# liubingqi7/audio-motion-avatar

Hardware: AMD Instinct MI355X
Metric: rendered frames/sec @512x512, 10k Gaussians (static triplane decode + SMPL-X LBS + tile rasterize) (higher is better)
Workload: dtype f32 (LBS blend-shape product: fp16 x 2 split operands with fp32 accumulation, fp32-equivalent; everything else plain fp32)

## Files before the change

audio-motion-avatar_amd/csrc/rasterizer.hip:

```cpp
#include <algorithm>
#include <cmath>
#include <cstddef>
#include <cstdlib>

#include "amav_common.h"
#include "decode_quad.h"
#include "raster_project.h"
#include "raster_workspace.h"

namespace amav {
namespace raster {

#ifndef AMAV_BIN_ABLATE
#define AMAV_BIN_ABLATE 0
#endif
#ifndef AMAV_ABLATE
#define AMAV_ABLATE 0
#endif
constexpr int kRenderWavesPerSimd = 4;
constexpr int kFusedMinFrames = 96;
constexpr int kSortCap = 512;
constexpr int kBigLdsCap = 2048;
constexpr int kBigBlocks = 1280;

constexpr int kQueues = 8;
constexpr int kBuckets = 17;

__host__ __device__ inline int bucket_of(int n) { return n > 512 ? 0 : 16 - (n - 1) / 32; }

struct Status {
    long long total;
    long long max_frame;
    long long emitted;
    int overflow;
    int big_count;
    int qcount[kQueues][kBuckets];
    int nempty;
    int next[kQueues][32];
};

struct Buffers {
    float4 *geom;
    uint4 *rectd;
    int *tile_off;
    unsigned long long *keys;
    unsigned *sorted;
    int *big_list;
    int4 *queue;
    int *empty_list;
    int *slice_counts;
    Status *status;
};

static inline int bin_slices(int F) { return F >= kFusedMinFrames ? 0 : std::min(16, std::max(1, (256 + F - 1) / F)); }

static inline size_t queue_capacity(int F, int gx, int gy) { return (size_t)F * ((gy + kQueues - 1) / kQueues) * gx; }

static Buffers carve(void *ws, int F, int N, int gx, int gy, long long cap, size_t *bytes) {
    const int T = gx * gy;
    Carver c(ws);
    Buffers b;
    b.status = c.take<Status>(1);
    b.geom = c.take<float4>(((size_t)F * N + 1024) * 3);
    b.rectd = c.take<uint4>((size_t)F * N + 1024);
    b.tile_off = c.take<int>((size_t)F * (T + 1));
    b.keys = c.take<unsigned long long>((size_t)cap);
    b.sorted = c.take<unsigned>((size_t)cap);
    b.big_list = c.take<int>((size_t)F * T);
    b.queue = c.take<int4>((size_t)kQueues * kBuckets * queue_capacity(F, gx, gy));
    b.empty_list = c.take<int>((size_t)F * T);
    b.slice_counts = c.take<int>((size_t)F * bin_slices(F) * T);
    if (bytes) *bytes = c.total();
    return b;
}

struct Params {
    int F, N, H, W, gx, gy, T;
    amav_attr means3d, rotations, scales, opacities, colors;
    const float *view, *proj, *tanfov;
    float bg[3];
    float scale_modifier;
    int apply_activations;
    float scale_bias, scale_max, opacity_bias;
    int antialiasing, clamp_output;
    float *out_rgba;
    float *out_inv_depth;
    int *out_radii;
    long long cap_per_frame;
    int qcap;
    unsigned long long *stamps;
    int *wire_header, *wire_frame_counts, *wire_offsets;
    unsigned char *wire_payload;
    int wire_cap;
    unsigned wire_bg;
    int stash;
    int slices;
    Buffers buf;
    struct {
        const float4 *proj;
        const float *vertices;
        const int *idx4;
        const float *transl;
        const float4 *wpoint;
        float4 *out;
        float radius;
        int R, V;
        int rec_lds;
    } dec;
};

__device__ __forceinline__ int opaque(int x) {
    asm volatile("" : "+v"(x));
    return x;
}
__device__ __forceinline__ int lane_now() {
    int l;
    asm volatile("v_mbcnt_lo_u32_b32 %0, -1, 0\n\tv_mbcnt_hi_u32_b32 %0, -1, %0" : "=v"(l));
    return l;
}
__device__ __forceinline__ unsigned zero_now() {
    unsigned z;
    asm volatile("v_mov_b32 %0, 0" : "=v"(z));
    return z;
}

__device__ __forceinline__ void wave_sync() {
    __builtin_amdgcn_fence(__ATOMIC_RELEASE, "wavefront");
    __builtin_amdgcn_wave_barrier();
    __builtin_amdgcn_fence(__ATOMIC_ACQUIRE, "wavefront");
}

struct GaussRec {
    float4 r0, r1, r2, r3;
};

template <bool kPacked>
__device__ __forceinline__ GaussRec load_gaussian(const Params &p, int f, int i) {
    GaussRec g;
    if (kPacked) {
        const float4 *rec = reinterpret_cast<const float4 *>(at(p.means3d, f, i));
        g.r0 = rec[0], g.r1 = rec[1], g.r2 = rec[2], g.r3 = rec[3];
    } else {
        const float *m_ = at(p.means3d, f, i), *q_ = at(p.rotations, f, i), *s_ = at(p.scales, f, i);
        const float *c_ = at(p.colors, f, i);
        g.r0 = make_float4(m_[0], m_[1], m_[2], at(p.opacities, f, i)[0]);
        g.r1 = make_float4(q_[0], q_[1], q_[2], q_[3]);
        g.r2 = make_float4(s_[0], s_[1], s_[2], 0.f);
        g.r3 = make_float4(c_[0], c_[1], c_[2], 0.f);
    }
    return g;
}

struct FrameCamera {
    float vm[16], pm[16];
    float tanx, tany;
};
__device__ __forceinline__ FrameCamera load_camera(const Params &p, int f) {
    FrameCamera c;
    auto uniform = [](float v) { return __uint_as_float(__builtin_amdgcn_readfirstlane(__float_as_uint(v))); };
#pragma unroll
    for (int k = 0; k < 16; ++k) c.vm[k] = uniform(p.view[f * 16 + k]), c.pm[k] = uniform(p.proj[f * 16 + k]);
    c.tanx = uniform(p.tanfov[2 * f]), c.tany = uniform(p.tanfov[2 * f + 1]);
    return c;
}

__device__ __forceinline__ uint4 preprocess_one(const Params &p, const GaussRec &rec, const FrameCamera &cam,
                                                int &upstream_tiles, float4 (&g)[3]) {
#pragma clang fp contract(off)
    const float *vm = cam.vm, *pm = cam.pm;
    const float tanx = cam.tanx, tany = cam.tany;
    uint4 rd = make_uint4(0u, 0u, 0u, 0u);
    const float4 rec0 = rec.r0, rec1 = rec.r1, rec2 = rec.r2, rec3 = rec.r3;
    const float px3 = rec0.x, py3 = rec0.y, pz3 = rec0.z;
    const ViewPoint v = view_point(vm, px3, py3, pz3);
    const float vx = v.x, vy = v.y, vz = v.z;
    if (!(vz > 0.2f)) return rd;
    const ClipPoint cp = clip_point(pm, px3, py3, pz3);
    const float ppx = cp.ppx, ppy = cp.ppy;

    const float r = rec1.x, x = rec1.y, y = rec1.z, z = rec1.w;
    float s0 = rec2.x, s1 = rec2.y, s2 = rec2.z;
    float opacity = rec0.w;
    float c0 = rec3.x, c1 = rec3.y, c2 = rec3.z;
    if (p.apply_activations) {
        float e;
        s0 = scale_act(s0, p.scale_bias, p.scale_max, e);
        s1 = scale_act(s1, p.scale_bias, p.scale_max, e);
        s2 = scale_act(s2, p.scale_bias, p.scale_max, e);
        opacity = opacity_act(opacity, p.opacity_bias);
        c0 = fminf(fmaxf(c0, 0.0f), 1.0f);
        c1 = fminf(fmaxf(c1, 0.0f), 1.0f);
        c2 = fminf(fmaxf(c2, 0.0f), 1.0f);
    }
    s0 *= p.scale_modifier;
    s1 *= p.scale_modifier;
    s2 *= p.scale_modifier;

    const Cov3 cv = cov3d(r, x, y, z, s0, s1, s2);

    const float focal_x = (float)p.W / (2.0f * tanx), focal_y = (float)p.H / (2.0f * tany);
    const float limx = 1.3f * tanx, limy = 1.3f * tany;
    const float tz = vz;
    const float tx = fminf(limx, fmaxf(-limx, vx / tz)) * tz;
    const float ty = fminf(limy, fmaxf(-limy, vy / tz)) * tz;
    const float J00 = focal_x / tz, J02 = -(focal_x * tx) / (tz * tz);
    const float J11 = focal_y / tz, J12 = -(focal_y * ty) / (tz * tz);
    float T0[3], T1[3];
#pragma unroll
    for (int b = 0; b < 3; ++b) {
        T0[b] = J00 * vm[b * 4 + 0] + J02 * vm[b * 4 + 2];
        T1[b] = J11 * vm[b * 4 + 1] + J12 * vm[b * 4 + 2];
    }
    const Cov2 cov = cov2d(cv.S, T0, T1);
    float ca = cov.ca;
    const float cb = cov.cb;
    float cc = cov.cc;

    const float det_cov = ca * cc - cb * cb;
    ca += 0.3f;
    cc += 0.3f;
    const float det = ca * cc - cb * cb;
    float h_scale = 1.0f;
    if (p.antialiasing) h_scale = sqrtf(fmaxf(0.000025f, det_cov / det));
    if (!(det > 0.0f)) return rd;
    const float det_inv = 1.0f / det;
    const float mid = 0.5f * (ca + cc);
    const float root = sqrtf(fmaxf(0.1f, mid * mid - det));
    const float my_radius = ceilf(3.0f * sqrtf(fmaxf(mid + root, mid - root)));
    const float pix_x = ((ppx + 1.0f) * (float)p.W - 1.0f) * 0.5f;
    const float pix_y = ((ppy + 1.0f) * (float)p.H - 1.0f) * 0.5f;
    const int rx0 = min(p.gx, max(0, (int)((pix_x - my_radius) / (float)kTile)));
    const int ry0 = min(p.gy, max(0, (int)((pix_y - my_radius) / (float)kTile)));
    const int rx1 = min(p.gx, max(0, (int)((pix_x + my_radius + (float)(kTile - 1)) / (float)kTile)));
    const int ry1 = min(p.gy, max(0, (int)((pix_y + my_radius + (float)(kTile - 1)) / (float)kTile)));
    if ((rx1 - rx0) * (ry1 - ry0) <= 0) return rd;

    const float op = opacity * h_scale;
    const float tau = 2.0f * logf(255.0f * op);
    float bx = -1e30f, by = -1e30f;
    if (tau > 0.0f) {
        bx = sqrtf(tau * ca) * 1.001f + 0.01f;
        by = sqrtf(tau * cc) * 1.001f + 0.01f;
    }
    upstream_tiles = (rx1 - rx0) * (ry1 - ry0);
    int cx0 = 1, cx1 = 0, cy0 = 1, cy1 = 0;
    if (tau > 0.0f) {
        cx0 = max(rx0, (int)floorf((pix_x - bx) / (float)kTile));
// ... 702 lines not shown
                   (base + c[4]) | ((base + c[5]) << 16), (base + c[6]) | ((base + c[7]) << 16));
    if (lane == 0) cnt[kBuckets512 / 2] = (unsigned)n;
    wave_sync();
    unsigned st[KPL], sz[KPL];
#pragma unroll
    for (int m = 0; m < KPL; ++m) {
        st[m] = (cnt[b[m] >> 1] >> (16 * (b[m] & 1))) & 0xffffu;
        const int nb = b[m] + 1;
        sz[m] = ((cnt[nb >> 1] >> (16 * (nb & 1))) & 0xffffu) - st[m];
        if (lane + 64 * m < n) slice[st[m] + pos[m]] = k[m];
    }
    wave_sync();
#pragma unroll
    for (int m = 0; m < KPL; ++m) {
        unsigned r = pos[m];
        if (lane + 64 * m < n && sz[m] > 1u) {
            r = 0;
            for (unsigned j = 0; j < sz[m]; ++j) r += (unsigned)(slice[st[m] + j] < k[m]);
        }
        pos[m] = st[m] + r;
    }
    wave_sync();
#pragma unroll
    for (int m = 0; m < KPL; ++m)
        if (lane + 64 * m < n) order[pos[m]] = (unsigned)k[m];
    wave_sync();
    return true;
}

__device__ __attribute__((noinline)) void wave_bitonic_sort(unsigned long long *a, unsigned *order, int n, int lane) {
    const int lp = 32 - __builtin_clz(n - 1);
    const int half = 1 << (lp - 1);
    auto cmpswap = [&](int lo, int hi) {
        if (hi < n) {
            const unsigned long long x = a[lo], y = a[hi];
            if (x > y) {
                a[lo] = y;
                a[hi] = x;
            }
        }
    };
    for (int lk = 1; lk <= lp; ++lk) {
        const int k = 1 << lk, hk = k >> 1;
        for (int c = lane; c < half; c += 64) {
            const int base = (c >> (lk - 1)) << lk, o = c & (hk - 1);
            cmpswap(base + o, base + k - 1 - o);
        }
        wave_sync();
        for (int lj = lk - 2; lj >= 0; --lj) {
            const int j = 1 << lj;
            for (int c = lane; c < half; c += 64) {
                const int lo = ((c >> lj) << (lj + 1)) + (c & (j - 1));
                cmpswap(lo, lo + j);
            }
            wave_sync();
        }
    }
    unsigned id[kSortCap / 64];
#pragma unroll
    for (int m = 0; m < kSortCap / 64; ++m) id[m] = (lane + 64 * m < n) ? (unsigned)a[lane + 64 * m] : 0u;
    wave_sync();
#pragma unroll
    for (int m = 0; m < kSortCap / 64; ++m)
        if (lane + 64 * m < n) order[lane + 64 * m] = id[m];
    wave_sync();
}

#define AMAV_BLEND_GEO(k0, k1, qa, qb, qc, L)           \
    "v_fma_f32 v92, -" qb ", %[ly], " k0 "\n\t"                                                                    \
    "v_fma_f32 v93, -" qc ", %[ly], " k1 "\n\t"                                                                    \
    "v_fma_f32 v92, -" qa ", %[lx], v92\n\t"                                                                       \
    "v_fma_f32 v92, -v92, v92, " L "\n\t"
#define AMAV_BLEND_REST(r, g, b, d, col_wait, DEPTH)                                                               \
    "v_fma_f32 v92, -v93, v93, v92\n\t"                                                                            \
    "v_exp_f32_e32 v92, v92\n\t"                                                                                   \
    "s_nop 0\n\t"                                                                                                  \
    "v_min_f32_e32 v92, 0x3f7d70a4, v92\n\t"                                                    \
    "v_cmp_le_f32_e32 vcc, 0x3b808081, v92\n\t"                                               \
    "s_nop 1\n\t"                                                                                                  \
    "v_cndmask_b32_e32 v92, 0, v92, vcc\n\t"                                       \
    "v_fma_f32 v93, -v92, %[T], %[T]\n\t"                                                   \
    "v_cmp_gt_f32_e32 vcc, 0x38d1b717, v93\n\t"                                          \
    "v_mul_f32_e32 v94, v92, %[T]\n\t"                                                        \
    "s_nop 0\n\t"                                                                                                  \
    "v_cndmask_b32_e64 v94, v94, 0, vcc\n\t"                                                                       \
    "v_cndmask_b32_e64 %[T], v93, -|%[T]|, vcc\n\t"                                                                \
    col_wait                                                                                                       \
    "v_fmac_f32_e32 %[R], " r ", v94\n\t"                                                                          \
    "v_fmac_f32_e32 %[G], " g ", v94\n\t"                                                                          \
    "v_fmac_f32_e32 %[B], " b ", v94\n\t" DEPTH(d)
#define AMAV_DEPTH_ON(d) "v_fmac_f32_e32 %[D], " d ", v94\n\t"
#define AMAV_DEPTH_OFF(d)
#define AMAV_BLEND_PAIR(use_x, use_y, load, DEPTH)                                                                 \
    "ds_read_b64 " load ", %[list] offset:16\n\t"                                                                  \
    "v_add_u32_e32 %[list], 8, %[list]\n\t"                                                                        \
    "s_waitcnt lgkmcnt(5)\n\t"                                                                                     \
    AMAV_BLEND_GEO("v68", "v69", "v70", "v71", "v72", "v73")                                                       \
    "ds_read_b128 v[68:71], " use_x "\n\t"                                                                         \
    "ds_read_b64 v[72:73], " use_x " offset:2080\n\t"                                                              \
    AMAV_BLEND_REST("v74", "v75", "v76", "v77", "s_waitcnt lgkmcnt(6)\n\t", DEPTH)                                 \
    "ds_read_b128 v[74:77], " use_x " offset:1040\n\t"                                                             \
    "s_waitcnt lgkmcnt(5)\n\t"                                                                                     \
    AMAV_BLEND_GEO("v78", "v79", "v80", "v81", "v82", "v83")                                                       \
    "ds_read_b128 v[78:81], " use_y "\n\t"                                                                         \
    "ds_read_b64 v[82:83], " use_y " offset:2080\n\t"                                                              \
    AMAV_BLEND_REST("v84", "v85", "v86", "v87", "s_waitcnt lgkmcnt(6)\n\t", DEPTH)                                 \
    "ds_read_b128 v[84:87], " use_y " offset:1040\n\t"
#define AMAV_BLEND_LOOP(DEPTH)                                                                                     \
    "s_waitcnt lgkmcnt(0)\n\t"                           \
    "ds_read_b64 v[88:89], %[list]\n\t"                                                                            \
    "ds_read_b64 v[90:91], %[list] offset:8\n\t"                                                                   \
    "s_waitcnt lgkmcnt(1)\n\t"                                                                                     \
    "ds_read_b128 v[68:71], v88\n\t"                                                                               \
    "ds_read_b64 v[72:73], v88 offset:2080\n\t"                                                                    \
    "ds_read_b128 v[74:77], v88 offset:1040\n\t"                                                                   \
    "ds_read_b128 v[78:81], v89\n\t"                                                                               \
    "ds_read_b64 v[82:83], v89 offset:2080\n\t"                                                                    \
    "ds_read_b128 v[84:87], v89 offset:1040\n\t"                                                                   \
    "1:\n\t"                                                                                                       \
    AMAV_BLEND_PAIR("v90", "v91", "v[88:89]", DEPTH)                                                               \
    "s_sub_u32 %[groups], %[groups], 1\n\t"                                                                        \
    "s_cmp_eq_u32 %[groups], 0\n\t"                                                                                \
    "s_cbranch_scc1 2f\n\t"                                                                                        \
    AMAV_BLEND_PAIR("v88", "v89", "v[90:91]", DEPTH)                                                               \
    "v_cmp_lt_f32_e32 vcc, 0, %[T]\n\t"                     \
    "s_sub_u32 %[groups], %[groups], 1\n\t"                                                                        \
    "s_cmp_eq_u32 %[groups], 0\n\t"                                                                                \
    "s_cbranch_scc1 2f\n\t"                                                                                        \
    "s_cbranch_vccnz 1b\n\t"                                                                                       \
    "2:\n\t"                                                                                                       \
    "s_waitcnt lgkmcnt(0)\n\t"
#define AMAV_BLEND_CLOBBERS                                                                                        \
    "memory", "vcc", "scc", "v68", "v69", "v70", "v71", "v72", "v73", "v74", "v75", "v76", "v77", "v78", "v79",    \
        "v80", "v81", "v82", "v83", "v84", "v85", "v86", "v87", "v88", "v89", "v90", "v91", "v92", "v93", "v94"

template <bool kInvDepth>
__device__ __forceinline__ bool blend_quadrant(unsigned list, int groups, float lx, float ly, float &T, float &R,
                                               float &G, float &B, float &D) {
    if (kInvDepth)
        asm volatile(AMAV_BLEND_LOOP(AMAV_DEPTH_ON)
                     : [T] "+v"(T), [R] "+v"(R), [G] "+v"(G), [B] "+v"(B), [D] "+v"(D), [list] "+v"(list), [groups] "+s"(groups)
                     : [lx] "v"(lx), [ly] "v"(ly)
                     : AMAV_BLEND_CLOBBERS);
    else
        asm volatile(AMAV_BLEND_LOOP(AMAV_DEPTH_OFF)
                     : [T] "+v"(T), [R] "+v"(R), [G] "+v"(G), [B] "+v"(B), [list] "+v"(list), [groups] "+s"(groups)
                     : [lx] "v"(lx), [ly] "v"(ly)
                     : AMAV_BLEND_CLOBBERS);
    return __any(T > 0.f);
}

#define AMAV_STAMP(slot)                                                                              \
    do {                                                                                              \
        if (p.stamps && lane == 0) p.stamps[(size_t)item * 6 + (slot)] = __builtin_amdgcn_s_memrealtime(); \
    } while (0)

typedef float nt_f4 __attribute__((ext_vector_type(4)));
__device__ __forceinline__ void store_nt(float *rgba, long long pid, float4 v) {
    const nt_f4 x = {v.x, v.y, v.z, v.w};
    __builtin_nontemporal_store(x, reinterpret_cast<nt_f4 *>(rgba) + pid);
}

struct FillCursor {
    int next, end;
    int have, pos;
    long long origin;
    int xy;
};

__device__ __forceinline__ void fill_fetch(const Params &p, FillCursor &c, int lane) {
    c.have = min(64, c.end - c.next);
    c.pos = 0;
    if (c.have <= 0) return;
    const int item = p.buf.empty_list[c.next + min(lane, c.have - 1)];
    c.next += c.have;
    const int f = item / p.T, t = item - f * p.T;
    const int ty = t / p.gx, tx = t - ty * p.gx;
    c.xy = (tx * kTile) | ((ty * kTile) << 16);
    c.origin = ((long long)f * p.H + ty * kTile) * p.W + tx * kTile;
}

template <bool kInvDepth>
__device__ __forceinline__ void fill_some(const Params &p, FillCursor &c, int count, int lane) {
    float r = p.bg[0], g = p.bg[1], bl = p.bg[2];
    if (p.clamp_output) {
        r = fminf(fmaxf(r, 0.f), 1.f);
        g = fminf(fmaxf(g, 0.f), 1.f);
        bl = fminf(fmaxf(bl, 0.f), 1.f);
    }
    const float4 px_bg = make_float4(r, g, bl, 0.0f);
    lane = opaque(lane);
    const int cx = lane & 15, cy = lane >> 4;
    while (count > 0) {
        if (c.pos >= c.have) {
            if (c.next >= c.end) return;
            fill_fetch(p, c, lane);
        }
        const int todo = min(count, c.have - c.pos);
        for (int j = c.pos; j < c.pos + todo; ++j) {
            const int xy = __builtin_amdgcn_readlane(c.xy, j);
            const long long origin = ((long long)__builtin_amdgcn_readlane((int)(c.origin >> 32), j) << 32) |
                                     (unsigned)__builtin_amdgcn_readlane((int)c.origin, j);
            const int X0 = xy & 0xffff, Y0 = xy >> 16;
            const bool in_x = X0 + cx < p.W;
#pragma unroll
            for (int k = 0; k < 4; ++k) {
                if (in_x && Y0 + cy + 4 * k < p.H) {
                    const long long pid = origin + (long long)(cy + 4 * k) * p.W + cx;
                    store_nt(p.out_rgba, pid, px_bg);
                    if (kInvDepth) p.out_inv_depth[pid] = 0.0f;
                }
            }
        }
        c.pos += todo;
        count -= todo;
    }
}

template <bool kInvDepth>
__device__ __forceinline__ void fill_tile_at(const Params &p, FillCursor &c, int lane) {
    const int j = c.pos++;
    const int xy = __builtin_amdgcn_readlane(c.xy, j);
    const long long origin = ((long long)__builtin_amdgcn_readlane((int)(c.origin >> 32), j) << 32) |
                             (unsigned)__builtin_amdgcn_readlane((int)c.origin, j);
    const int X0 = xy & 0xffff, Y0 = xy >> 16;
    float r = p.bg[0], g = p.bg[1], bl = p.bg[2];
    if (p.clamp_output) {
        r = fminf(fmaxf(r, 0.f), 1.f);
        g = fminf(fmaxf(g, 0.f), 1.f);
        bl = fminf(fmaxf(bl, 0.f), 1.f);
    }
    const int cx = lane & 15, cy = lane >> 4;
    const bool in_x = X0 + cx < p.W;
#pragma unroll
    for (int k = 0; k < 4; ++k) {
        if (in_x && Y0 + cy + 4 * k < p.H) {
            const long long pid = origin + (long long)(cy + 4 * k) * p.W + cx;
            store_nt(p.out_rgba, pid, make_float4(r, g, bl, 0.0f));
            if (kInvDepth) p.out_inv_depth[pid] = 0.0f;
        }
    }
}

struct TileRef {
    int item, beg, n;
    int slot;
};

constexpr int kPrepCap = 256;
constexpr int kPrepBuckets = 256;

__device__ __forceinline__ void sort_prefetched(const unsigned long long (&k)[4], int n, unsigned long long *slice,
                                                unsigned *cnt, unsigned *order, int lane) {
    if (n <= 64) {
        if (lane < n) slice[lane] = k[0];
        wave_sync();
        rank_sort<1>(slice, order, n, lane);
        return;
    }
    unsigned dmin = 0xffffffffu, dmax = 0u;
#pragma unroll
    for (int m = 0; m < 4; ++m) {
        const unsigned d = (unsigned)(k[m] >> 32);
        if (lane + 64 * m < n) dmin = min(dmin, d), dmax = max(dmax, d);
    }
    dmin = wave_min_u32(dmin), dmax = wave_max_u32(dmax);
    const float scale = dmax > dmin ? (float)(kPrepBuckets - 1) / (float)(dmax - dmin) : 0.0f;
    int b[4];
#pragma unroll
    for (int m = 0; m < 4; ++m) b[m] = min(kPrepBuckets - 1, (int)((float)((unsigned)(k[m] >> 32) - dmin) * scale));
    {
        const unsigned z = zero_now();
        reinterpret_cast<uint2 *>(cnt)[lane] = make_uint2(z, z);
    }
    wave_sync();
    unsigned pos[4];
#pragma unroll
    for (int m = 0; m < 4; ++m) {
        pos[m] = 0;
        if (lane + 64 * m < n) {
            const int sh = 16 * (b[m] & 1);
            pos[m] = (atomicAdd(&cnt[b[m] >> 1], 1u << sh) >> sh) & 0xffffu;
        }
    }
    wave_sync();
    const uint2 w = reinterpret_cast<uint2 *>(cnt)[lane];
    unsigned c[4] = {w.x & 0xffffu, w.x >> 16, w.y & 0xffffu, w.y >> 16};
    unsigned tot = 0, big = 0;
#pragma unroll
    for (int i = 0; i < 4; ++i) {
        const unsigned ci = c[i];
        big = max(big, ci);
        c[i] = tot;
        tot += ci;
    }
    const unsigned incl = wave_inclusive_sum_u32(tot, lane);
    big = wave_max_u32(big);
    if (big > (unsigned)kBucketMax) {
        wave_sync();
#pragma unroll
        for (int m = 0; m < 4; ++m)
            if (lane + 64 * m < n) slice[lane + 64 * m] = k[m];
        wave_sync();
        rank_sort<4>(slice, order, n, lane);
        return;
    }
    const unsigned base = incl - tot;
    reinterpret_cast<uint2 *>(cnt)[lane] = make_uint2((base + c[0]) | ((base + c[1]) << 16), (base + c[2]) | ((base + c[3]) << 16));
    if (lane == 0) cnt[kPrepBuckets / 2] = (unsigned)n;
    wave_sync();
    unsigned st[4], sz[4];
#pragma unroll
    for (int m = 0; m < 4; ++m) {
        st[m] = (cnt[b[m] >> 1] >> (16 * (b[m] & 1))) & 0xffffu;
        const int nb = b[m] + 1;
        sz[m] = ((cnt[nb >> 1] >> (16 * (nb & 1))) & 0xffffu) - st[m];
        if (lane + 64 * m < n) slice[st[m] + pos[m]] = k[m];
    }
    wave_sync();
#pragma unroll
    for (int m = 0; m < 4; ++m) {
        unsigned r = pos[m];
        if (lane + 64 * m < n && sz[m] > 1u) {
            r = 0;
            for (unsigned j = 0; j < sz[m]; ++j) r += (unsigned)(slice[st[m] + j] < k[m]);
        }
        pos[m] = st[m] + r;
    }
    wave_sync();
#pragma unroll
    for (int m = 0; m < 4; ++m)
        if (lane + 64 * m < n) order[pos[m]] = (unsigned)k[m];
    wave_sync();
}

template <bool kInvDepth>
__global__ __launch_bounds__(64, kRenderWavesPerSimd) void render_kernel(Params p) {
    __shared__ WaveLds lds;
    WaveLds &L = lds;
    const int lane = threadIdx.x;
    const Status *st = p.buf.status;
    const int q = blockIdx.x % kQueues, stride = gridDim.x / kQueues;
    FillCursor fill;
    {
        const int nempty = st->nempty;
        const int per = (nempty + (int)gridDim.x - 1) / (int)gridDim.x;
        fill.next = min(nempty, (int)blockIdx.x * per);
        fill.end = min(nempty, fill.next + per);
        fill.have = fill.pos = 0;
        fill.origin = 0, fill.xy = 0;
    }
    int bucket_end = (lane < kBuckets && !st->overflow) ? st->qcount[q][lane] : 0;
#pragma unroll
    for (int d = 1; d < 32; d <<= 1) {
        const int o = __shfl_up(bucket_end, d, 64);
        if (lane >= d) bucket_end += o;
    }
    const int total = __builtin_amdgcn_readlane(bucket_end, kBuckets - 1);
    if (lane < 32) L.bucket_end[lane] = bucket_end;
    wave_sync();
    int i_cur = blockIdx.x / kQueues;
    if (i_cur < total) {
        const int expect = max(1, (total + stride - 1) / stride);
        const int fill_chunk = (fill.end - fill.next + expect - 1) / expect;
        int *next = const_cast<int *>(&st->next[q][0]);
        const int4 *queue_q = p.buf.queue + (size_t)q * kBuckets * p.qcap;
        auto entry_of = [&](int i) {
            const int l = lane_now();
            const int b = __popcll(__ballot(l < kBuckets && i >= L.bucket_end[l & 31]));
            const int first = b > 0 ? L.bucket_end[b - 1] : 0;
            return queue_q + (size_t)b * p.qcap + (i - __builtin_amdgcn_readfirstlane(first));
        };
        unsigned *order_l = reinterpret_cast<unsigned *>(L.keys);
        typedef __attribute__((address_space(3))) const unsigned lds_u32;
        lds_u32 *order_lds = (lds_u32 *)order_l;
        unsigned *prep_cnt = reinterpret_cast<unsigned *>(&L.keys[kSortCap / 2]);
        const unsigned stage_base = (unsigned)(uintptr_t)(__attribute__((address_space(3))) void *)&L.geo[0];
        const unsigned lists_base = (unsigned)(uintptr_t)(__attribute__((address_space(3))) void *)&L.keys[kSortCap / 2];
        const unsigned null_slot = stage_base + (unsigned)kNullSlot * 16u;
        auto write_null_record = [&]() {
            if (lane_now() == 0) {
                const float z = __uint_as_float(zero_now());
                L.geo[kNullSlot] = make_float4(z, z, z, z);
                L.col[kNullSlot] = make_float4(z, z, z, z);
                L.geo2[kNullSlot] = make_float4(z, -__builtin_inff(), z, z);
            }
        };
        write_null_record();
#if AMAV_ABLATE != 5 && AMAV_ABLATE != 7
        fill_fetch(p, fill, lane);
#endif
        int idx_v = 0;
        if (lane == 0) idx_v = stride + atomicAdd(next, 1);
        const int4 e0 = *entry_of(i_cur);
        TileRef cur = {__builtin_amdgcn_readfirstlane(e0.x), __builtin_amdgcn_readfirstlane(e0.y),
                       __builtin_amdgcn_readfirstlane(e0.z), __builtin_amdgcn_readfirstlane(e0.w)};
        bool ready = false;
        float4 g0 = make_float4(0.f, 0.f, 0.f, 0.f), g1 = g0, g2 = g0;
        int i_next = __builtin_amdgcn_readfirstlane(idx_v);
        int4 e_next = make_int4(0, 0, 0, 0);
        if (i_next < total) e_next = *entry_of(i_next);
        for (;;) {
            const int ln = lane_now();
            int idx2 = 0;
            if (ln == 0) idx2 = stride + atomicAdd(next, 1);
            int4 e_after = make_int4(0, 0, 0, 0);
            const int item = cur.item, n = cur.n;
            const unsigned my_slot = stage_base + (unsigned)ln * 16u;
            const int f = item / p.T, t = item - f * p.T;
            AMAV_STAMP(0);
            const int tx = t % p.gx, ty = t / p.gx;
            const int X0 = tx * kTile, Y0 = ty * kTile;
            const unsigned *order_g = p.buf.sorted + (size_t)f * p.cap_per_frame + cur.beg;
            const float4 *geom = p.buf.geom + (size_t)f * p.N * 3;
            const bool local = n <= kSortCap;
            if (p.stamps && ln == 0) p.stamps[(size_t)item * 6 + 5] = (unsigned long long)n;
            auto load_records = [&](int k) {
                unsigned id;
                if (local)
                    id = order_lds[k];
                else
                    id = order_g[k];
                const float4 *g = geom + (size_t)id * 3;
                g0 = g[0], g1 = g[1], g2 = g[2];
            };
#ifndef AMAV_STAMP_DETAIL
            AMAV_STAMP(1);
#endif
#ifdef AMAV_STAMP_DETAIL
            const unsigned long long own_0 = __builtin_amdgcn_s_memrealtime();
#endif
            if (!ready) {
                const unsigned long long *keys = p.buf.keys + (size_t)f * p.cap_per_frame + cur.beg;
                if (local) {
                    unsigned *cnt = reinterpret_cast<unsigned *>(L.geo);
                    bool done = false;
                    if (n <= 64) {
                        for (int k = ln; k < n; k += 64) L.keys[k] = keys[k];
                        wave_sync();
                    } else if (n <= 128)
                        done = bucket_sort<2>(keys, L.keys, cnt, order_l, n, ln);
                    else if (n <= 192)
                        done = bucket_sort<3>(keys, L.keys, cnt, order_l, n, ln);
                    else if (n <= 256)
                        done = bucket_sort<4>(keys, L.keys, cnt, order_l, n, ln);
                    else if (n <= 384)
                        done = bucket_sort<6>(keys, L.keys, cnt, order_l, n, ln);
                    else
                        done = bucket_sort<8>(keys, L.keys, cnt, order_l, n, ln);
                    if (!done) {
                        if (n <= 64)
                            rank_sort<1>(L.keys, order_l, n, ln);
                        else if (n <= 128)
                            rank_sort<2>(L.keys, order_l, n, ln);
                        else if (n <= 192)
                            rank_sort<3>(L.keys, order_l, n, ln);
                        else if (n <= 256)
                            rank_sort<4>(L.keys, order_l, n, ln);
                        else
                            wave_bitonic_sort(L.keys, order_l, n, ln);
                    }
                    write_null_record();
                }
                if (ln < n) load_records(ln);
            }
            AMAV_STAMP(2);

            const int lx = ln & 7, ly = ln >> 3;
            float lxf0 = (float)lx, lxf1 = (float)(8 + lx), lyf0 = (float)ly, lyf1 = (float)(8 + ly);
            asm volatile("" : "+v"(lxf0), "+v"(lxf1), "+v"(lyf0), "+v"(lyf1));
            const bool in0 = X0 + lx < p.W, in1 = X0 + 8 + lx < p.W, inr0 = Y0 + ly < p.H, inr1 = Y0 + 8 + ly < p.H;
            float T0 = (in0 & inr0) ? 1.f : -1.f, T1 = (in1 & inr0) ? 1.f : -1.f;
            float T2 = (in0 & inr1) ? 1.f : -1.f, T3 = (in1 & inr1) ? 1.f : -1.f;
            float R0 = 0.f, G0 = 0.f, B0 = 0.f, D0 = 0.f, R1 = 0.f, G1 = 0.f, B1 = 0.f, D1 = 0.f;
            float R2 = 0.f, G2 = 0.f, B2 = 0.f, D2 = 0.f, R3 = 0.f, G3 = 0.f, B3 = 0.f, D3 = 0.f;
            const float X0f = (float)X0, Y0f = (float)Y0;

            TileRef nxt = {0, 0, 0, 0};
            bool ready_next = false;
            const float4 *geom_next = geom;

#ifdef AMAV_STAMP_DETAIL
            unsigned long long t_asm = 0, t_fill = 0, t_prep = 0, t_stage = 0, t_own = __builtin_amdgcn_s_memrealtime() - own_0;
#define AMAV_TIC(x) const unsigned long long x##_0 = __builtin_amdgcn_s_memrealtime()
#define AMAV_TOC(x, acc) acc += __builtin_amdgcn_s_memrealtime() - x##_0
#else
#define AMAV_TIC(x)
#define AMAV_TOC(x, acc)
#endif
            int qalive = 15;
            int fill_left = fill_chunk;
            const int fill_round = (fill_chunk * 64 + n - 1) / max(n, 64) + 0;
            for (int base = 0;; base += 64) {
                const bool more = qalive != 0 && base < n;
                const bool last = !more || base + 64 >= n;
                int n0 = 0, n1 = 0, n2 = 0, n3 = 0;
                unsigned long long pk[4] = {~0ull, ~0ull, ~0ull, ~0ull};
                unsigned idf = 0;
                if (last) {
                    nxt.item = __builtin_amdgcn_readfirstlane(e_next.x);
                    nxt.beg = __builtin_amdgcn_readfirstlane(e_next.y);
                    nxt.n = __builtin_amdgcn_readfirstlane(e_next.z);
                    nxt.slot = __builtin_amdgcn_readfirstlane(e_next.w);
                    if (nxt.n > 0) {
                        const int fn = nxt.item / p.T;
                        geom_next = p.buf.geom + (size_t)fn * p.N * 3;
                        if (nxt.n <= kPrepCap) {
                            const unsigned long long *kn = p.buf.keys + (size_t)fn * p.cap_per_frame + nxt.beg;
#pragma unroll
                            for (int m = 0; m < 4; ++m)
                                if (ln + 64 * m < nxt.n) pk[m] = kn[ln + 64 * m];
                        } else if (nxt.n > kSortCap) {
                            if (ln < nxt.n) idf = p.buf.sorted[(size_t)fn * p.cap_per_frame + nxt.beg + ln];
                        }
                    }
                }
                if (more) {
                    AMAV_TIC(s0);
                    int qm = 0;
                    if (base + ln < n) {
                        qm = quad_mask(g0, g2, X0f, Y0f) & qalive;
                    }
                    if (qm != 0) {
                        const float2 k = tile_k(g0, g1, X0f, Y0f);
                        L.geo[ln] = make_float4(k.x, k.y, g0.z, g0.w);
                        *reinterpret_cast<float2 *>(&L.geo2[ln]) = make_float2(g1.x, g1.y);
                        L.col[ln] = make_float4(g1.z, g1.w, g2.x, g2.y);
                    }
                    const unsigned long long m0 = __ballot(qm & 1), m1 = __ballot(qm & 2), m2 = __ballot(qm & 4),
                                             m3 = __ballot(qm & 8);
                    n0 = __popcll(m0), n1 = __popcll(m1), n2 = __popcll(m2), n3 = __popcll(m3);
                    auto put = [&](int qd, unsigned long long m, int cnt, int bit) {
                        typedef __attribute__((address_space(3))) unsigned lds_u32w;
                        lds_u32w *list = (lds_u32w *)(uintptr_t)(lists_base + (unsigned)qd * (kListStride * 4u));
                        if (qm & bit)
                            list[__builtin_amdgcn_mbcnt_hi((unsigned)(m >> 32), __builtin_amdgcn_mbcnt_lo((unsigned)m, 0u))] = my_slot;
                        if (ln < kListTail) list[cnt + ln] = null_slot;
                    };
                    if (n0) put(0, m0, n0, 1);
                    if (n1) put(1, m1, n1, 2);
                    if (n2) put(2, m2, n2, 4);
                    if (n3) put(3, m3, n3, 8);
                    wave_sync();
                    AMAV_TOC(s0, t_stage);
#if AMAV_ABLATE != 5 && AMAV_ABLATE != 7
                    { AMAV_TIC(f0);
                    for (int k = 0; k < fill_round && fill_left > 0 && fill.pos < fill.have; ++k, --fill_left)
                        fill_tile_at<kInvDepth>(p, fill, ln);
                    AMAV_TOC(f0, t_fill); }
#endif
                    if (!last && base + 64 + ln < n) load_records(base + 64 + ln);
#if AMAV_ABLATE != 3 && AMAV_ABLATE != 7
                    { AMAV_TIC(a0);
                    if (n0 && !blend_quadrant<kInvDepth>(lists_base, (n0 + 1) >> 1, lxf0, lyf0, T0, R0, G0, B0, D0)) qalive &= ~1;
                    AMAV_TOC(a0, t_asm); }
#endif
                }
                if (base == 0) {
                    i_next = __builtin_amdgcn_readfirstlane(idx2);
                    if (i_next < total) e_after = *entry_of(i_next);
                }
#if AMAV_ABLATE != 3 && AMAV_ABLATE != 7
                if (more) {
                    AMAV_TIC(a1);
                    if (n1 && !blend_quadrant<kInvDepth>(lists_base + kListStride * 4u, (n1 + 1) >> 1, lxf1, lyf0, T1, R1, G1, B1, D1)) qalive &= ~2;
                    AMAV_TOC(a1, t_asm);
                }
#endif
                if (last) {
                    AMAV_TIC(p0);
                    if (nxt.n > 0 && nxt.n <= kPrepCap) {
                        sort_prefetched(pk, nxt.n, L.keys, prep_cnt, order_l, ln);
                        if (ln < nxt.n) {
                            const float4 *g = geom_next + (size_t)order_lds[ln] * 3;
                            g0 = g[0], g1 = g[1], g2 = g[2];
                        }
                        ready_next = true;
                    } else if (nxt.n > kSortCap) {
                        if (ln < nxt.n) {
                            const float4 *g = geom_next + (size_t)idf * 3;
                            g0 = g[0], g1 = g[1], g2 = g[2];
                        }
                        ready_next = true;
                    }
                    AMAV_TOC(p0, t_prep);
                }
#if AMAV_ABLATE != 3 && AMAV_ABLATE != 7
                if (more) {
                    AMAV_TIC(a2);
                    if (n2 && !blend_quadrant<kInvDepth>(lists_base + kListStride * 8u, (n2 + 1) >> 1, lxf0, lyf1, T2, R2, G2, B2, D2)) qalive &= ~4;
                    if (n3 && !blend_quadrant<kInvDepth>(lists_base + kListStride * 12u, (n3 + 1) >> 1, lxf1, lyf1, T3, R3, G3, B3, D3)) qalive &= ~8;
                    AMAV_TOC(a2, t_asm);
                }
#endif

                wave_sync();
                if (last) break;
            }
            asm volatile("s_waitcnt vmcnt(0)"
                         : "+v"(g0.x), "+v"(g0.y), "+v"(g0.z), "+v"(g0.w), "+v"(g1.x), "+v"(g1.y), "+v"(g1.z), "+v"(g1.w),
                           "+v"(g2.x), "+v"(g2.y), "+v"(g2.z), "+v"(g2.w)
                         :
                         : "memory");

#ifdef AMAV_STAMP_DETAIL
            if (p.stamps && lane == 0) {
                p.stamps[(size_t)item * 6 + 1] = t_asm;
                p.stamps[(size_t)item * 6 + 2] = (t_prep << 48) | ((t_fill & 0xffffull) << 32) | ((t_stage & 0xffffull) << 16) | (t_own & 0xffffull);
            }
#endif
            AMAV_STAMP(3);
            {
                const float Tq[4] = {fabsf(T0), fabsf(T1), fabsf(T2), fabsf(T3)};
                const float Rq[4] = {R0, R1, R2, R3}, Gq[4] = {G0, G1, G2, G3}, Bq[4] = {B0, B1, B2, B3}, Dq[4] = {D0, D1, D2, D3};
#pragma unroll
                for (int qd = 0; qd < 4; ++qd) {
                    const int px = X0 + 8 * (qd & 1) + lx, py = Y0 + 8 * (qd >> 1) + ly;
                    if (px < p.W && py < p.H) {
                        float r = Rq[qd] + Tq[qd] * p.bg[0], g = Gq[qd] + Tq[qd] * p.bg[1], bl = Bq[qd] + Tq[qd] * p.bg[2];
                        if (p.clamp_output) {
                            r = fminf(fmaxf(r, 0.f), 1.f);
                            g = fminf(fmaxf(g, 0.f), 1.f);
                            bl = fminf(fmaxf(bl, 0.f), 1.f);
                        }
                        const size_t pid = ((size_t)f * p.H + py) * p.W + px;
                        store_nt(p.out_rgba, pid, make_float4(r, g, bl, 1.0f - Tq[qd]));
                        if (kInvDepth) p.out_inv_depth[pid] = Dq[qd];
                    }
                }
                if (p.wire_header && cur.slot < p.wire_cap) {
                    unsigned char *bytes = reinterpret_cast<unsigned char *>(L.geo);
                    const unsigned bgw = p.wire_bg;
#pragma unroll
                    for (int qd = 0; qd < 4; ++qd) {
                        const int tx16 = 8 * (qd & 1) + lx, ty16 = 8 * (qd >> 1) + ly;
                        unsigned cr = bgw & 255u, cg = (bgw >> 8) & 255u, cb = (bgw >> 16) & 255u;
                        if (X0 + tx16 < p.W && Y0 + ty16 < p.H) {
                            const float r = Rq[qd] + Tq[qd] * p.bg[0], g = Gq[qd] + Tq[qd] * p.bg[1], bl = Bq[qd] + Tq[qd] * p.bg[2];
                            cr = (unsigned)(unsigned char)(fminf(fmaxf(r, 0.f), 1.f) * 255.0f);
                            cg = (unsigned)(unsigned char)(fminf(fmaxf(g, 0.f), 1.f) * 255.0f);
                            cb = (unsigned)(unsigned char)(fminf(fmaxf(bl, 0.f), 1.f) * 255.0f);
                        }
                        unsigned char *px3 = bytes + (ty16 * 16 + tx16) * 3;
                        px3[0] = (unsigned char)cr, px3[1] = (unsigned char)cg, px3[2] = (unsigned char)cb;
                    }
                    wave_sync();
                    const unsigned *words = reinterpret_cast<const unsigned *>(bytes) + ln * 3;
                    const unsigned w0 = words[0], w1 = words[1], w2 = words[2];
                    unsigned *dst = reinterpret_cast<unsigned *>(p.wire_payload + (size_t)cur.slot * kWireTileBytes) + ln * 3;
                    dst[0] = w0, dst[1] = w1, dst[2] = w2;
                    wave_sync();
                }
            }
            AMAV_STAMP(4);
#if AMAV_ABLATE != 5 && AMAV_ABLATE != 7
            if (fill_left > 0 || fill.pos >= fill.have) fill_some<kInvDepth>(p, fill, fill_left, ln);
            if (fill.pos >= fill.have && fill.next < fill.end) fill_fetch(p, fill, ln);
#endif
            if (nxt.n <= 0) break;
            cur = nxt;
            ready = ready_next;
            e_next = e_after;
        }
    }
#if AMAV_ABLATE != 5 && AMAV_ABLATE != 7
    fill_some<kInvDepth>(p, fill, 0x7fffffff, lane_now());
#endif
}

}
}

using namespace amav;
using namespace amav::raster;

static unsigned render_grid(bool ) {
    static unsigned g = 0;
    if (g) return g;
    int dev = 0, cus = 256;
    if (hipGetDevice(&dev) != hipSuccess || hipDeviceGetAttribute(&cus, hipDeviceAttributeMultiprocessorCount, dev) != hipSuccess || cus <= 0)
        cus = 256;
    (void)hipGetLastError();
    int per_cu = 4 * kRenderWavesPerSimd;
    if (const char *env = getenv("AMAV_RENDER_WAVES")) {
        const int v = atoi(env);
        if (v >= 1 && v <= 32) per_cu = v;
    }
    g = (unsigned)(cus * per_cu) / kQueues * kQueues;
    if (g < (unsigned)kQueues) g = kQueues;
    return g;
}

extern "C" size_t amav_rasterize_workspace_bytes(int F, int N, int H, int W, int64_t capacity) {
    if (F <= 0 || N <= 0 || H <= 0 || W <= 0 || capacity < 0) return 0;
    const int gx = (W + kTile - 1) / kTile, gy = (H + kTile - 1) / kTile;
    size_t bytes = 0;
    carve(nullptr, F, N, gx, gy, capacity / F * F, &bytes);
    return bytes;
}

static int rasterize_forward(const amav_raster_args *a, const amav_decode_source *d, void *stream_) {
    AMAV_REQUIRE(a != nullptr, "amav_rasterize_forward: args is NULL");
    AMAV_REQUIRE(a->num_frames > 0 && a->num_gaussians > 0 && a->height > 0 && a->width > 0,
                 "amav_rasterize_forward: bad sizes F=%d N=%d H=%d W=%d", a->num_frames, a->num_gaussians, a->height,
                 a->width);
    AMAV_REQUIRE(a->means3d.ptr && a->rotations.ptr && a->scales.ptr && a->opacities.ptr && a->colors.ptr,
                 "amav_rasterize_forward: NULL Gaussian attribute");
    AMAV_REQUIRE(a->viewmatrix && a->projmatrix && a->tanfov, "amav_rasterize_forward: NULL camera");
    AMAV_REQUIRE(a->out_rgba != nullptr, "amav_rasterize_forward: out_rgba is NULL");
    AMAV_REQUIRE(a->workspace != nullptr, "amav_rasterize_forward: workspace is NULL");
    AMAV_REQUIRE(a->instance_capacity >= 0, "amav_rasterize_forward: negative instance_capacity");
    AMAV_REQUIRE((reinterpret_cast<uintptr_t>(a->out_rgba) & 15) == 0, "amav_rasterize_forward: out_rgba not 16-B aligned");
    const int F = a->num_frames, N = a->num_gaussians;
    const int gx = (a->width + kTile - 1) / kTile, gy = (a->height + kTile - 1) / kTile;
    AMAV_REQUIRE(gx < 65536 && gy < 65536, "amav_rasterize_forward: image too large");
    const int T = gx * gy;
    AMAV_REQUIRE((long long)F * T < (1ll << 31), "amav_rasterize_forward: F * tiles overflows int32");
    const size_t bin_lds = ((size_t)2 * T + 48 + 3 * kQueues * (kBuckets + 1)) * sizeof(int);
    AMAV_REQUIRE(bin_lds <= 160 * 1024, "amav_rasterize_forward: %d tiles need %zu B of LDS in the binning block (max 160 KiB)",
                 T, bin_lds);
    const bool stash = bin_lds + 8 + (size_t)N * 8 <= 160 * 1024 && gx <= 255 && gy <= 255 && a->out_radii == nullptr;
    const size_t rec_lds = align_up(bin_lds + (size_t)N * 8, 16);
    const bool fits_decode = stash && rec_lds + 1024 * 64 <= 160 * 1024;
    const long long cap_per_frame = a->instance_capacity / F;
    AMAV_REQUIRE(cap_per_frame < (1ll << 31), "amav_rasterize_forward: per-frame instance capacity overflows int32");
    size_t need = 0;
    Params p;
    p.dec = {};
    p.buf = carve(a->workspace, F, N, gx, gy, cap_per_frame * F, &need);
    if (a->workspace_bytes < need)
        return fail(AMAV_ERR_WORKSPACE, "amav_rasterize_forward: workspace %zu < required %zu", a->workspace_bytes, need);
    p.F = F, p.N = N, p.H = a->height, p.W = a->width, p.gx = gx, p.gy = gy, p.T = T;
    p.means3d = a->means3d, p.rotations = a->rotations, p.scales = a->scales, p.opacities = a->opacities;
    p.colors = a->colors;
    p.view = a->viewmatrix, p.proj = a->projmatrix, p.tanfov = a->tanfov;
    p.bg[0] = a->bg[0], p.bg[1] = a->bg[1], p.bg[2] = a->bg[2];
    p.scale_modifier = a->scale_modifier;
    p.apply_activations = a->apply_activations;
    p.scale_bias = a->scale_bias, p.scale_max = a->scale_max, p.opacity_bias = a->opacity_bias;
    p.antialiasing = a->antialiasing, p.clamp_output = a->clamp_output;
    p.out_rgba = a->out_rgba, p.out_inv_depth = a->out_inv_depth, p.out_radii = a->out_radii;
    p.cap_per_frame = cap_per_frame;
    p.qcap = (int)queue_capacity(F, gx, gy);
    p.stamps = static_cast<unsigned long long *>(a->debug_stamps);
    p.wire_header = nullptr, p.wire_frame_counts = nullptr, p.wire_offsets = nullptr, p.wire_payload = nullptr;
    p.wire_cap = 0, p.wire_bg = 0;
    p.slices = bin_slices(F);
    p.stash = stash ? 1 : 0;
    if (a->wire) {
        AMAV_REQUIRE(a->clamp_output, "amav_rasterize_forward: the wire output carries the clamped colours (set clamp_output)");
        AMAV_REQUIRE((reinterpret_cast<uintptr_t>(a->wire) & 15) == 0 && a->wire_capacity_tiles >= 0 &&
                         a->wire_capacity_tiles <= (long long)F * T,
                     "amav_rasterize_forward: bad wire buffer (alignment, or capacity %lld outside [0, %lld])",
                     (long long)a->wire_capacity_tiles, (long long)F * T);
        const size_t wire_need = (wire_payload_at(F, F * T) + (size_t)a->wire_capacity_tiles * kWireTileBytes + 15) / 16 * 16;
        if (a->wire_bytes < wire_need)
            return fail(AMAV_ERR_WORKSPACE, "amav_rasterize_forward: wire buffer %zu < required %zu", a->wire_bytes, wire_need);
        p.wire_header = static_cast<int *>(a->wire);
        p.wire_frame_counts = p.wire_header + kWireHeaderInts;
        p.wire_offsets = p.wire_frame_counts + F;
        p.wire_payload = static_cast<unsigned char *>(a->wire) + wire_payload_at(F, F * T);
        p.wire_cap = (int)a->wire_capacity_tiles;
        auto q8 = [](float v) { return (unsigned)(unsigned char)(std::fmin(std::fmax(v, 0.f), 1.f) * 255.0f); };
        p.wire_bg = q8(a->bg[0]) | (q8(a->bg[1]) << 8) | (q8(a->bg[2]) << 16);
    }

    hipStream_t stream = static_cast<hipStream_t>(stream_);
    static const hipError_t attr[6] = {
        hipFuncSetAttribute(reinterpret_cast<const void *>(&slice_count_kernel), hipFuncAttributeMaxDynamicSharedMemorySize, 160 * 1024),
        hipFuncSetAttribute(reinterpret_cast<const void *>(&slice_scatter_kernel), hipFuncAttributeMaxDynamicSharedMemorySize, 160 * 1024),
        hipFuncSetAttribute(reinterpret_cast<const void *>(&bin_kernel<true, false>), hipFuncAttributeMaxDynamicSharedMemorySize, 160 * 1024),
        hipFuncSetAttribute(reinterpret_cast<const void *>(&bin_kernel<true, true>), hipFuncAttributeMaxDynamicSharedMemorySize, 160 * 1024),
        hipFuncSetAttribute(reinterpret_cast<const void *>(&bin_kernel<false, false>), hipFuncAttributeMaxDynamicSharedMemorySize, 160 * 1024),
        hipFuncSetAttribute(reinterpret_cast<const void *>(&bin_kernel<true, true, true>), hipFuncAttributeMaxDynamicSharedMemorySize, 160 * 1024)};
    if (attr[0] != hipSuccess || attr[1] != hipSuccess || attr[2] != hipSuccess || attr[3] != hipSuccess || attr[4] != hipSuccess ||
        attr[5] != hipSuccess)
        return fail(AMAV_ERR_LAUNCH, "amav_rasterize_forward: cannot raise the dynamic LDS limit");
    const float *b0 = a->means3d.ptr;
    const bool packed = (reinterpret_cast<uintptr_t>(b0) & 15) == 0 && a->means3d.elem_stride == 16 &&
                        a->means3d.frame_stride % 4 == 0 && a->opacities.ptr == b0 + 3 && a->rotations.ptr == b0 + 4 &&
                        a->scales.ptr == b0 + 8 && a->colors.ptr == b0 + 12 && a->opacities.elem_stride == 16 &&
                        a->rotations.elem_stride == 16 && a->scales.elem_stride == 16 && a->colors.elem_stride == 16 &&
                        a->opacities.frame_stride == a->means3d.frame_stride &&
                        a->rotations.frame_stride == a->means3d.frame_stride &&
                        a->scales.frame_stride == a->means3d.frame_stride &&
                        a->colors.frame_stride == a->means3d.frame_stride;
    const bool decode_fused = d && F >= kFusedMinFrames && fits_decode;
    if (d) {
        AMAV_REQUIRE(packed && a->means3d.frame_stride == (int64_t)N * 16,
                     "amav_rasterize_decode_forward: the Gaussian attributes must view one contiguous packed [F, N, 16] buffer");
        AMAV_REQUIRE(d->resolution > 0 && d->num_verts > 0 && d->radius > 0.0f,
                     "amav_rasterize_decode_forward: bad decode source (R=%d V=%d radius=%g)", d->resolution, d->num_verts,
                     (double)d->radius);
        AMAV_REQUIRE(d->proj && d->vertices && d->idx4 && d->head_w_point,
                     "amav_rasterize_decode_forward: NULL decode input");
        AMAV_REQUIRE(((reinterpret_cast<uintptr_t>(d->proj) | reinterpret_cast<uintptr_t>(d->idx4) |
                       reinterpret_cast<uintptr_t>(d->head_w_point)) & 15) == 0,
                     "amav_rasterize_decode_forward: proj/idx4/head_w_point not 16-B aligned");
        p.dec.proj = reinterpret_cast<const float4 *>(d->proj);
        p.dec.vertices = d->vertices;
        p.dec.idx4 = d->idx4;
        p.dec.transl = d->transl;
        p.dec.wpoint = reinterpret_cast<const float4 *>(d->head_w_point);
        p.dec.out = reinterpret_cast<float4 *>(const_cast<float *>(b0));
        p.dec.radius = d->radius;
        p.dec.R = d->resolution, p.dec.V = d->num_verts;
        p.dec.rec_lds = (int)rec_lds;
        if (!decode_fused) {
            const int rc = amav_triplane_sample_decode_indexed(F, N, d->resolution, d->num_verts, d->proj, d->vertices,
                                                               d->idx4, d->transl, d->radius, d->head_w_point,
                                                               const_cast<float *>(b0), stream);
            if (rc != AMAV_OK) return rc;
        }
    }
    if (zero_async(p.buf.status, sizeof(Status), stream) != hipSuccess)
        return fail(AMAV_ERR_LAUNCH, "amav_rasterize_forward: status clear failed");
    if (p.wire_header && zero_async(p.wire_header, (size_t)kWireHeaderInts * 4, stream) != hipSuccess)
        return fail(AMAV_ERR_LAUNCH, "amav_rasterize_forward: wire header clear failed");

    if (F < kFusedMinFrames && F <= 65535) {
        const dim3 pre_grid((unsigned)((N + 255) / 256), (unsigned)F);
        if (packed)
            preprocess_kernel<true><<<pre_grid, 256, 0, stream>>>(p);
        else
            preprocess_kernel<false><<<pre_grid, 256, 0, stream>>>(p);
        const dim3 slice_grid((unsigned)p.slices, (unsigned)F);
        slice_count_kernel<<<slice_grid, 1024, (size_t)T * sizeof(int), stream>>>(p);
        bin_kernel<false, false><<<F, 1024, bin_lds, stream>>>(p);
        slice_scatter_kernel<<<slice_grid, 1024, (size_t)T * sizeof(int), stream>>>(p);
    } else if (decode_fused)
        bin_kernel<true, true, true><<<F, 1024, rec_lds + 1024 * 64, stream>>>(p);
    else if (packed)
        bin_kernel<true, true><<<F, 1024, bin_lds + (stash ? 8 + (size_t)N * 8 : 0), stream>>>(p);
    else
        bin_kernel<true, false><<<F, 1024, bin_lds + (stash ? 8 + (size_t)N * 8 : 0), stream>>>(p);
    sort_big_kernel<<<kBigBlocks, 256, 0, stream>>>(p);
    const unsigned blocks = render_grid(a->out_inv_depth != nullptr);
    if (a->profile_start_event) (void)hipEventRecord(static_cast<hipEvent_t>(a->profile_start_event), stream);
    if (a->out_inv_depth)
        render_kernel<true><<<blocks, 64, 0, stream>>>(p);
    else
        render_kernel<false><<<blocks, 64, 0, stream>>>(p);
    if (a->profile_stop_event) (void)hipEventRecord(static_cast<hipEvent_t>(a->profile_stop_event), stream);
    return check_launch("amav_rasterize_forward");
}

extern "C" int amav_rasterize_forward(const amav_raster_args *a, void *stream) { return rasterize_forward(a, nullptr, stream); }

extern "C" int amav_rasterize_decode_forward(const amav_raster_args *a, const amav_decode_source *d, void *stream) {
    AMAV_REQUIRE(d != nullptr, "amav_rasterize_decode_forward: decode source is NULL");
    return rasterize_forward(a, d, stream);
}

namespace amav {
namespace raster {
__global__ __launch_bounds__(256) void tile_counts_kernel(int F, int T, const Status *__restrict__ st,
                                                          const int *__restrict__ tile_off, int *__restrict__ out) {
    const int i = blockIdx.x * blockDim.x + threadIdx.x;
    if (i >= F * T) return;
    const int f = i / T, t = i - f * T;
    const int *off = tile_off + (size_t)f * (T + 1);
    out[i] = st->overflow ? 1 : off[t + 1] - off[t];
}

WorkspaceView workspace_view(void *workspace, int F, int N, int H, int W, long long instance_capacity) {
    const int gx = (W + kTile - 1) / kTile, gy = (H + kTile - 1) / kTile;
    const long long cap_per_frame = instance_capacity / F;
    size_t bytes = 0;
    const Buffers b = carve(workspace, F, N, gx, gy, cap_per_frame * F, &bytes);
    WorkspaceView v;
    v.geom = b.geom, v.rectd = b.rectd, v.tile_off = b.tile_off, v.keys = b.keys, v.sorted = b.sorted;
    v.overflow = workspace ? &b.status->overflow : nullptr;
    v.cap_per_frame = cap_per_frame;
    v.sort_cap = kSortCap;
    v.bytes = bytes;
    return v;
}
}
}

extern "C" int amav_rasterize_tile_counts(const void *workspace, int F, int N, int H, int W, int64_t capacity,
                                          int32_t *out_counts, void *stream_) {
    AMAV_REQUIRE(workspace && out_counts, "amav_rasterize_tile_counts: NULL pointer");
    AMAV_REQUIRE(F > 0 && N > 0 && H > 0 && W > 0 && capacity >= 0, "amav_rasterize_tile_counts: bad sizes");
    const int gx = (W + kTile - 1) / kTile, gy = (H + kTile - 1) / kTile, T = gx * gy;
    size_t bytes = 0;
    const Buffers b = carve(const_cast<void *>(workspace), F, N, gx, gy, capacity / F * F, &bytes);
    tile_counts_kernel<<<(unsigned)(((long long)F * T + 255) / 256), 256, 0, static_cast<hipStream_t>(stream_)>>>(
        F, T, b.status, b.tile_off, out_counts);
    return check_launch("amav_rasterize_tile_counts");
}

extern "C" int amav_rasterize_status(const void *workspace, int64_t *total, int64_t *max_frame, int32_t *overflow,
                                     void *stream_) {
    AMAV_REQUIRE(workspace != nullptr, "amav_rasterize_status: workspace is NULL");
    Status s;
    hipStream_t stream = static_cast<hipStream_t>(stream_);
    hipError_t e = hipMemcpyAsync(&s, workspace, sizeof(Status), hipMemcpyDeviceToHost, stream);
    if (e == hipSuccess) e = hipStreamSynchronize(stream);
    if (e != hipSuccess) return fail(AMAV_ERR_LAUNCH, "amav_rasterize_status: %s", hipGetErrorString(e));
    if (total) *total = s.total;
// ... 5 lines not shown
```

Before: 320,300.

## Split long-list render tiles into per-quadrant work items for load balance

When a queue holds long tile lists (bucket 0) or the total queued work is light relative to the number of render waves, each long-list tile is expanded into four work items, one per 8x8 quadrant. The quadrant mask gates blending and output, so the longest tiles are spread across several waves and the tail imbalance shrinks. The cost is that staging the tile's Gaussian list and the prep work now run four times for those tiles. The split is on by default and can be controlled with the AMAV_RENDER_SPLIT environment variable.

```diff
diff --git a/audio-motion-avatar_amd/csrc/rasterizer.hip b/audio-motion-avatar_amd/csrc/rasterizer.hip
--- a/audio-motion-avatar_amd/csrc/rasterizer.hip
+++ b/audio-motion-avatar_amd/csrc/rasterizer.hip
@@ -23,6 +23,7 @@
 constexpr int kBigLdsCap = 2048;
 constexpr int kBigBlocks = 1280;
 
+constexpr int kRenderSplit = 1;
 constexpr int kQueues = 8;
 constexpr int kBuckets = 17;
 
@@ -93,6 +94,7 @@
     unsigned char *wire_payload;
     int wire_cap;
     unsigned wire_bg;
+    int split;
     int stash;
     int slices;
     Buffers buf;
@@ -1101,7 +1103,7 @@
 
 #define AMAV_STAMP(slot)                                                                              \
     do {                                                                                              \
-        if (p.stamps && lane == 0) p.stamps[(size_t)item * 6 + (slot)] = __builtin_amdgcn_s_memrealtime(); \
+        if (p.stamps && lane == 0 && (quads & 1)) p.stamps[(size_t)item * 6 + (slot)] = __builtin_amdgcn_s_memrealtime(); \
     } while (0)
 
 typedef float nt_f4 __attribute__((ext_vector_type(4)));
@@ -1300,6 +1302,14 @@
         fill.origin = 0, fill.xy = 0;
     }
     int bucket_end = (lane < kBuckets && !st->overflow) ? st->qcount[q][lane] : 0;
+    const int long_lists = __builtin_amdgcn_readlane(bucket_end, 0);
+    float queued = (float)bucket_end * (lane == 0 ? 1024.0f : (float)(32 * (kBuckets - lane)));
+#pragma unroll
+    for (int d = 32; d >= 1; d >>= 1) queued += __shfl_xor(queued, d, 64);
+    queued = __int_as_float(__builtin_amdgcn_readfirstlane(__float_as_int(queued)));
+    const bool split_queue = p.split > 0 && (long_lists > stride || queued <= 512.0f * (float)p.split * (float)stride);
+    const int split_end = split_queue ? 4 * long_lists : 0;
+    if (lane == 0 && split_end) bucket_end = split_end;
 #pragma unroll
     for (int d = 1; d < 32; d <<= 1) {
         const int o = __shfl_up(bucket_end, d, 64);
@@ -1318,8 +1328,10 @@
             const int l = lane_now();
             const int b = __popcll(__ballot(l < kBuckets && i >= L.bucket_end[l & 31]));
             const int first = b > 0 ? L.bucket_end[b - 1] : 0;
-            return queue_q + (size_t)b * p.qcap + (i - __builtin_amdgcn_readfirstlane(first));
+            const int at = i - __builtin_amdgcn_readfirstlane(first);
+            return queue_q + (size_t)b * p.qcap + (i < split_end ? at >> 2 : at);
         };
+        auto quads_of = [&](int i) { return i < split_end ? 1 << (i & 3) : 15; };
         unsigned *order_l = reinterpret_cast<unsigned *>(L.keys);
         typedef __attribute__((address_space(3))) const unsigned lds_u32;
         lds_u32 *order_lds = (lds_u32 *)order_l;
@@ -1349,6 +1361,7 @@
         int i_next = __builtin_amdgcn_readfirstlane(idx_v);
         int4 e_next = make_int4(0, 0, 0, 0);
         if (i_next < total) e_next = *entry_of(i_next);
+        int quads = quads_of(i_cur) | (quads_of(i_next) << 4);
         for (;;) {
             const int ln = lane_now();
             int idx2 = 0;
@@ -1363,7 +1376,7 @@
             const unsigned *order_g = p.buf.sorted + (size_t)f * p.cap_per_frame + cur.beg;
             const float4 *geom = p.buf.geom + (size_t)f * p.N * 3;
             const bool local = n <= kSortCap;
-            if (p.stamps && ln == 0) p.stamps[(size_t)item * 6 + 5] = (unsigned long long)n;
+            if (p.stamps && ln == 0 && (quads & 1)) p.stamps[(size_t)item * 6 + 5] = (unsigned long long)n;
             auto load_records = [&](int k) {
                 unsigned id;
                 if (local)
@@ -1437,7 +1450,7 @@
 #define AMAV_TIC(x)
 #define AMAV_TOC(x, acc)
 #endif
-            int qalive = 15;
+            int qalive = quads & (1 | (X0 + 8 < p.W ? 2 : 0) | (Y0 + 8 < p.H ? (X0 + 8 < p.W ? 12 : 4) : 0));
             int fill_left = fill_chunk;
             const int fill_round = (fill_chunk * 64 + n - 1) / max(n, 64) + 0;
             for (int base = 0;; base += 64) {
@@ -1508,6 +1521,7 @@
                 if (base == 0) {
                     i_next = __builtin_amdgcn_readfirstlane(idx2);
                     if (i_next < total) e_after = *entry_of(i_next);
+                    quads |= quads_of(i_next) << 8;
                 }
 #if AMAV_ABLATE != 3 && AMAV_ABLATE != 7
                 if (more) {
@@ -1553,7 +1567,7 @@
                          : "memory");
 
 #ifdef AMAV_STAMP_DETAIL
-            if (p.stamps && lane == 0) {
+            if (p.stamps && lane == 0 && (quads & 1)) {
                 p.stamps[(size_t)item * 6 + 1] = t_asm;
                 p.stamps[(size_t)item * 6 + 2] = (t_prep << 48) | ((t_fill & 0xffffull) << 32) | ((t_stage & 0xffffull) << 16) | (t_own & 0xffffull);
             }
@@ -1565,7 +1579,7 @@
 #pragma unroll
                 for (int qd = 0; qd < 4; ++qd) {
                     const int px = X0 + 8 * (qd & 1) + lx, py = Y0 + 8 * (qd >> 1) + ly;
-                    if (px < p.W && py < p.H) {
+                    if (((quads >> qd) & 1) && px < p.W && py < p.H) {
                         float r = Rq[qd] + Tq[qd] * p.bg[0], g = Gq[qd] + Tq[qd] * p.bg[1], bl = Bq[qd] + Tq[qd] * p.bg[2];
                         if (p.clamp_output) {
                             r = fminf(fmaxf(r, 0.f), 1.f);
@@ -1580,9 +1594,11 @@
                 if (p.wire_header && cur.slot < p.wire_cap) {
                     unsigned char *bytes = reinterpret_cast<unsigned char *>(L.geo);
                     const unsigned bgw = p.wire_bg;
+                    const int wl = lane_now();
 #pragma unroll
                     for (int qd = 0; qd < 4; ++qd) {
-                        const int tx16 = 8 * (qd & 1) + lx, ty16 = 8 * (qd >> 1) + ly;
+                        if (!((quads >> qd) & 1)) continue;
+                        const int tx16 = 8 * (qd & 1) + (wl & 7), ty16 = 8 * (qd >> 1) + (wl >> 3);
                         unsigned cr = bgw & 255u, cg = (bgw >> 8) & 255u, cb = (bgw >> 16) & 255u;
                         if (X0 + tx16 < p.W && Y0 + ty16 < p.H) {
                             const float r = Rq[qd] + Tq[qd] * p.bg[0], g = Gq[qd] + Tq[qd] * p.bg[1], bl = Bq[qd] + Tq[qd] * p.bg[2];
@@ -1594,10 +1610,12 @@
                         px3[0] = (unsigned char)cr, px3[1] = (unsigned char)cg, px3[2] = (unsigned char)cb;
                     }
                     wave_sync();
-                    const unsigned *words = reinterpret_cast<const unsigned *>(bytes) + ln * 3;
-                    const unsigned w0 = words[0], w1 = words[1], w2 = words[2];
-                    unsigned *dst = reinterpret_cast<unsigned *>(p.wire_payload + (size_t)cur.slot * kWireTileBytes) + ln * 3;
-                    dst[0] = w0, dst[1] = w1, dst[2] = w2;
+                    if ((quads >> (((ln >> 5) << 1) | ((ln >> 1) & 1))) & 1) {
+                        const unsigned *words = reinterpret_cast<const unsigned *>(bytes) + ln * 3;
+                        const unsigned w0 = words[0], w1 = words[1], w2 = words[2];
+                        unsigned *dst = reinterpret_cast<unsigned *>(p.wire_payload + (size_t)cur.slot * kWireTileBytes) + ln * 3;
+                        dst[0] = w0, dst[1] = w1, dst[2] = w2;
+                    }
                     wave_sync();
                 }
             }
@@ -1610,10 +1628,17 @@
             cur = nxt;
             ready = ready_next;
             e_next = e_after;
-        }
-    }
+            quads >>= 4;
+        }
+    }
+#ifdef AMAV_STAMP_WAVES
+    if (p.stamps && lane == 0) p.stamps[(size_t)p.F * p.T * 6 + blockIdx.x * 2] = __builtin_amdgcn_s_memrealtime();
+#endif
 #if AMAV_ABLATE != 5 && AMAV_ABLATE != 7
     fill_some<kInvDepth>(p, fill, 0x7fffffff, lane_now());
+#endif
+#ifdef AMAV_STAMP_WAVES
+    if (p.stamps && lane == 0) p.stamps[(size_t)p.F * p.T * 6 + blockIdx.x * 2 + 1] = __builtin_amdgcn_s_memrealtime();
 #endif
 }
 
@@ -1638,6 +1663,14 @@
     g = (unsigned)(cus * per_cu) / kQueues * kQueues;
     if (g < (unsigned)kQueues) g = kQueues;
     return g;
+}
+
+static int render_split() {
+    if (const char *env = getenv("AMAV_RENDER_SPLIT")) {
+        const int v = atoi(env);
+        if (v >= 0 && v <= 1 << 20) return v;
+    }
+    return kRenderSplit;
 }
 
 extern "C" size_t amav_rasterize_workspace_bytes(int F, int N, int H, int W, int64_t capacity) {
@@ -1696,6 +1729,7 @@
     p.wire_cap = 0, p.wire_bg = 0;
     p.slices = bin_slices(F);
     p.stash = stash ? 1 : 0;
+    p.split = render_split();
     if (a->wire) {
         AMAV_REQUIRE(a->clamp_output, "amav_rasterize_forward: the wire output carries the clamped colours (set clamp_output)");
         AMAV_REQUIRE((reinterpret_cast<uintptr_t>(a->wire) & 15) == 0 && a->wire_capacity_tiles >= 0 &&
```

Result: no change. 319,800 (-0.2%).
